# underdoc-wang/STC-GNN

Hardware: AMD Instinct MI355X
Metric: STC-GNN fwd+bwd samples/sec at N=50k,C=32; SpMM HBM GB/s vs peak, 1/8 GPU (higher is better)
Workload: dtype f32; 1 GPU; full STC-GNN train step (fwd + ComboLoss + bwd + grad all-reduce + Adam), csr-fixed, 224x224 queen grid N=50176 nnz=398724, C=32, hidden=16, K=2, layers=2, T=18+6; global_batch=8, batch_per_gpu=8, parallelism=batch-shard x1, operand_format=f16x2, grad_bucket_bytes=88132, grad_large_bytes=0, input_seeds=X, Y: Bernoulli(0.1635), torch seed 1000 + rank

## Files before the change

stc-gnn_amd/csrc/stc_spmm_ring2.hip:

```cpp
#include "stc_spmm_host.h"

namespace {

constexpr int R2_THREADS = 256, R2_WAVES = R2_THREADS / 64;
constexpr int R2_INT = STC_RING2_INTERIOR;
constexpr int R2_L1 = STC_RING2_FIRST;
constexpr int R2_L2 = STC_RING2_SECOND;
constexpr int R2_W = STC_RING2_WIDTH;
constexpr int R2_Q = 32;
constexpr int R2_STAGE = R2_L2 / (2 * R2_WAVES);
constexpr int R2_S1 = R2_L1 / (2 * R2_WAVES);
constexpr int R2_S2 = R2_INT / (2 * R2_WAVES);
constexpr int R2_MAX_ADD = STC_RING2_MAX_ADD;

using v4f = __attribute__((ext_vector_type(4))) float;

struct Ring2Plan {
    const int32_t *l2_rows, *l1_rows, *int_rows;
    const int32_t *t1, *t2;
    int n_patches;
};

struct Ring2Args {
    Ring2Plan pl;
    const v4f *A, *A2;
    const v4f* add[R2_MAX_ADD];
    int n_add;
    const v4f *U, *Cand;
    v4f *Y, *Y2, *Z;
    int n, F4;
    float alpha1, alpha2;
    const v4f* add0[R2_MAX_ADD];
    float scale0[R2_MAX_ADD];
};

enum { R2_SUM = 0, R2_BLEND = 1, R2_CHAIN = 2, R2_BLEND0 = 3 };

__device__ __forceinline__ void lds_only_barrier() { asm volatile("s_waitcnt lgkmcnt(0)\n\ts_barrier" ::: "memory"); }

template <int MODE, bool HAS_A2, int NADD, int N0 = 0>
__global__ __launch_bounds__(R2_THREADS, 2) void ring2_sum_kernel(Ring2Args a) {
    static_assert((MODE != R2_BLEND && MODE != R2_BLEND0) || (NADD == 1 && !HAS_A2), "the blend forms: one addend (A), one gathered operand (Bm)");
    static_assert((MODE == R2_CHAIN) == (N0 > 0), "interior addends: the chain form, at least one");
    extern __shared__ __attribute__((aligned(16))) unsigned char lds[];
    v4f* tile = reinterpret_cast<v4f*>(lds);
    int2* tab1 = reinterpret_cast<int2*>(lds + (size_t)R2_L2 * R2_Q * 16);
    int2* tab2 = tab1 + R2_L1 * R2_W;

    const int p = stc_xcd_tile(blockIdx.x, a.pl.n_patches);
    if (p < 0) return;
    const int b = blockIdx.y;
    const int tid = threadIdx.x, lane = tid & 63, half = lane >> 5, q = lane & 31;
    const int wave = __builtin_amdgcn_readfirstlane(tid >> 6);
    const int hw = wave * 2 + half;
    const int n_chunks = a.F4 / R2_Q;

    for (int e = tid; e < R2_L1 * R2_W; e += R2_THREADS) tab1[e] = reinterpret_cast<const int2*>(a.pl.t1)[(size_t)p * R2_L1 * R2_W + e];
    for (int e = tid; e < R2_INT * R2_W; e += R2_THREADS) tab2[e] = reinterpret_cast<const int2*>(a.pl.t2)[(size_t)p * R2_INT * R2_W + e];

    int stage_row[R2_STAGE], l1_row[R2_S1], in_row[R2_S2];
#pragma unroll
    for (int k = 0; k < R2_STAGE; ++k) stage_row[k] = a.pl.l2_rows[(size_t)p * R2_L2 + k * 8 + hw];
#pragma unroll
    for (int i = 0; i < R2_S1; ++i) l1_row[i] = a.pl.l1_rows[(size_t)p * R2_L1 + i * 8 + hw];
#pragma unroll
    for (int i = 0; i < R2_S2; ++i) in_row[i] = a.pl.int_rows[(size_t)p * R2_INT + i * 8 + hw];

    const unsigned base = (unsigned)b * (unsigned)a.n * (unsigned)a.F4 + (unsigned)q;
    unsigned stage_off[R2_STAGE], l1_off[R2_S1];
#pragma unroll
    for (int k = 0; k < R2_STAGE; ++k) stage_off[k] = base + (unsigned)stage_row[k] * (unsigned)a.F4;
#pragma unroll
    for (int i = 0; i < R2_S1; ++i) l1_off[i] = base + (unsigned)(l1_row[i] >= 0 ? (l1_row[i] & 0x3FFFFFFF) : 0) * (unsigned)a.F4;
    v4f st[R2_STAGE];
    auto request = [&](int chunk) {
#pragma unroll
        for (int k = 0; k < R2_STAGE; ++k) {
            const unsigned at = stage_off[k] + chunk * R2_Q;
            st[k] = a.A[at];
            if (HAS_A2) st[k] += a.A2[at];
        }
    };
    constexpr int NOP = MODE == R2_CHAIN ? NADD : MODE == R2_BLEND0 ? NADD + 1 : NADD + 2, NOPA = NOP > 0 ? NOP : 1;
    auto slot_at = [&](int i, int chunk) { return l1_off[i] + (unsigned)(chunk * R2_Q); };
    auto request_slot = [&](v4f (&o)[NOPA], int i, int chunk) {
        const unsigned at = slot_at(i, chunk);
#pragma unroll
        for (int k = 0; k < NADD; ++k) o[k] = a.add[k][at];
        if constexpr (MODE != R2_CHAIN) {
            o[NADD] = a.U[at];
            if constexpr (MODE != R2_BLEND0) o[NADD + 1] = a.Cand[at];
        }
    };
    v4f opn[NOPA];
    request(0);
    request_slot(opn, 0, 0);
    for (int chunk = 0; chunk < n_chunks; ++chunk) {
        if (chunk) lds_only_barrier();
#pragma unroll
        for (int k = 0; k < R2_STAGE; ++k) tile[(k * 8 + hw) * R2_Q + q] = st[k];
        lds_only_barrier();
        const bool more = chunk + 1 < n_chunks;
        v4f dy[R2_S1];
#pragma unroll
        for (int i = 0; i < R2_S1; ++i) {
            const int slot = i * 8 + hw, row = l1_row[i];
            const bool interior = row >= 0 && (row & (1 << 30));
            v4f cur[NOPA];
#pragma unroll
            for (int k = 0; k < NOP; ++k) cur[k] = opn[k];
            if (i + 1 < R2_S1) {
                request_slot(opn, i + 1, chunk);
            } else if (more) {
                request(chunk + 1);
                request_slot(opn, 0, chunk + 1);
            }
            v4f acc = {0.f, 0.f, 0.f, 0.f};
#pragma unroll
            for (int w = 0; w < R2_W; ++w) {
                const int2 t = tab1[slot * R2_W + w];
                const v4f x = *reinterpret_cast<const v4f*>(lds + t.x + q * 16);
                const float v = __int_as_float(t.y);
#pragma unroll
                for (int c = 0; c < 4; ++c) acc[c] = fmaf(v, x[c], acc[c]);
            }
            v4f dh = MODE == R2_CHAIN ? a.alpha1 * acc : acc;
#pragma unroll
            for (int k = 0; k < NADD; ++k) dh += cur[k];
            if constexpr (MODE == R2_CHAIN) {
                if (a.Y != nullptr && interior) __builtin_nontemporal_store(dh, a.Y + slot_at(i, chunk));
                dy[i] = dh;
            } else if constexpr (MODE == R2_SUM) {
                const v4f u = cur[NOPA - 2], cd = cur[NOPA - 1];
                if (interior) __builtin_nontemporal_store(dh, a.Y + slot_at(i, chunk));
#pragma unroll
                for (int c = 0; c < 4; ++c) dy[i][c] = dh[c] * u[c] * (1.f - cd[c] * cd[c]);
            } else {
                const v4f u = cur[NADD], cd = MODE == R2_BLEND0 ? v4f{0.f, 0.f, 0.f, 0.f} : cur[NOPA - 1];
                v4f cand;
#pragma unroll
                for (int c = 0; c < 4; ++c) {
                    cand[c] = stc_tanh(dh[c]);
                    if constexpr (MODE == R2_BLEND0) dy[i][c] = u[c] * cand[c];
                    else dy[i][c] = (1.f - u[c]) * cd[c] + u[c] * cand[c];
                }
                if (interior) {
                    if (a.Y != nullptr) __builtin_nontemporal_store(cand, a.Y + slot_at(i, chunk));
                    __builtin_nontemporal_store(dy[i], a.Y2 + slot_at(i, chunk));
                }
            }
        }
        lds_only_barrier();
#pragma unroll
        for (int i = 0; i < R2_S1; ++i) tile[(i * 8 + hw) * R2_Q + q] = dy[i];
        v4f own[R2_S2][N0 > 0 ? N0 : 1];
        if constexpr (MODE == R2_CHAIN) {
#pragma unroll
            for (int i = 0; i < R2_S2; ++i)
#pragma unroll
                for (int k = 0; k < N0; ++k)
                    own[i][k] = a.add0[k][base + (unsigned)(in_row[i] >= 0 ? in_row[i] : 0) * (unsigned)a.F4 + (unsigned)(chunk * R2_Q)];
        }
        lds_only_barrier();
#pragma unroll
        for (int i = 0; i < R2_S2; ++i) {
            const int r = i * 8 + hw, row = in_row[i];
            v4f acc = {0.f, 0.f, 0.f, 0.f};
#pragma unroll
            for (int w = 0; w < R2_W; ++w) {
                const int2 t = tab2[r * R2_W + w];
                const v4f x = *reinterpret_cast<const v4f*>(lds + t.x + q * 16);
                const float v = __int_as_float(t.y);
#pragma unroll
                for (int c = 0; c < 4; ++c) acc[c] = fmaf(v, x[c], acc[c]);
            }
            if constexpr (MODE == R2_CHAIN) {
                acc *= a.alpha2;
#pragma unroll
                for (int k = 0; k < N0; ++k) acc += a.scale0[k] * own[i][k];
            }
            if (row >= 0) __builtin_nontemporal_store(acc, a.Z + (base + (unsigned)row * (unsigned)a.F4 + (unsigned)(chunk * R2_Q)));
        }
    }
}

template <int MODE, bool HAS_A2>
int launch_ring2(const Ring2Args& a, int batch, hipStream_t s, int n_add0 = 0) {
    const size_t lds = (size_t)R2_L2 * R2_Q * 16 + (size_t)(R2_L1 + R2_INT) * R2_W * sizeof(int2);
    static_assert((size_t)R2_L2 * R2_Q * 16 + (size_t)(R2_L1 + R2_INT) * R2_W * sizeof(int2) <= 64 * 1024, "within the default dynamic-LDS limit: no attribute to set");
    using Kernel = void (*)(Ring2Args);
    Kernel kern = nullptr;
    if constexpr (MODE == R2_BLEND || MODE == R2_BLEND0) {
        kern = ring2_sum_kernel<MODE, false, 1>;
    } else if constexpr (MODE == R2_CHAIN) {
        static constexpr Kernel table[3][R2_MAX_ADD] = {
#define STC_R2_ROW(NA) {ring2_sum_kernel<R2_CHAIN, HAS_A2, NA, 1>, ring2_sum_kernel<R2_CHAIN, HAS_A2, NA, 2>, ring2_sum_kernel<R2_CHAIN, HAS_A2, NA, 3>, \
                        ring2_sum_kernel<R2_CHAIN, HAS_A2, NA, 4>, ring2_sum_kernel<R2_CHAIN, HAS_A2, NA, 5>}
            STC_R2_ROW(0), STC_R2_ROW(1), STC_R2_ROW(2)};
#undef STC_R2_ROW
        kern = table[a.n_add][n_add0 - 1];
    } else {
        switch (a.n_add) {
            case 0: kern = ring2_sum_kernel<R2_SUM, HAS_A2, 0>; break;
            case 1: kern = ring2_sum_kernel<R2_SUM, HAS_A2, 1>; break;
            case 2: kern = ring2_sum_kernel<R2_SUM, HAS_A2, 2>; break;
            case 3: kern = ring2_sum_kernel<R2_SUM, HAS_A2, 3>; break;
            case 4: kern = ring2_sum_kernel<R2_SUM, HAS_A2, 4>; break;
            default: kern = ring2_sum_kernel<R2_SUM, HAS_A2, 5>; break;
        }
    }
    const int per = (a.pl.n_patches + stc::kNumXcd - 1) / stc::kNumXcd;
    hipLaunchKernelGGL(kern, dim3(per * stc::kNumXcd, batch), dim3(R2_THREADS), lds, s, a);
    return stc::launched("stc_ring2 launch");
}

int check_ring2(const char* who, const void* l2_rows, const void* l1_rows, const void* int_rows, const void* t1, const void* t2, int n_patches, int n_rows,
                int batch, int C, int h) {
    STC_REQUIRE(h == 16 && C >= 1 && (C * h) % (4 * R2_Q) == 0, STC_EUNSUPPORTED, "%s: rows of C * h = %d floats (hidden 16, whole 512-byte chunks)", who, C * h);
    STC_REQUIRE(batch <= 65535 && n_patches >= 0, STC_EINVAL, "%s: bad sizes", who);
    if (int rc = stc::check_state_rows(who, n_rows, batch, C, h, true)) return rc;
    STC_REQUIRE((long long)batch * n_rows * (C * h / 4) < (1ll << 28), STC_ELIMIT, "%s: planes of %lld 16-byte pieces (32-bit offsets: < 2^28)", who,
                (long long)batch * n_rows * (C * h / 4));
    if (batch == 0 || n_rows == 0) return STC_OK;
    STC_REQUIRE(n_patches >= 1 && (long long)n_patches * R2_INT >= n_rows, STC_EINVAL, "%s: %d patches cannot cover %d rows", who, n_patches, n_rows);
    STC_REQUIRE(l2_rows && l1_rows && int_rows && t1 && t2, STC_EINVAL, "%s: null plan array", who);
    STC_REQUIRE(reinterpret_cast<uintptr_t>(t1) % 8 == 0 && reinterpret_cast<uintptr_t>(t2) % 8 == 0, STC_EALIGN, "%s: tables must be 8-byte aligned", who);
    return STC_OK;
}

}

#if !defined(STC_RING2_FIRST_UNIT)

extern "C" int stc_ring2_sum_f32(const int32_t* l2_rows, const int32_t* l1_rows, const int32_t* int_rows, const int32_t* t1, const int32_t* t2,
                                 int32_t n_patches, int32_t n_rows,
                                 const float* A, const float* A2, int32_t n_add, const float* const* add,
                                 const float* U, const float* Cand, float* Y, float* Z,
                                 int32_t batch, int32_t C, int32_t h, void* stream) {
    if (int rc = stc::check_addend_count("stc_ring2_sum_f32", "addend", n_add, 0, R2_MAX_ADD, STC_ELIMIT)) return rc;
    if (int rc = check_ring2("stc_ring2_sum_f32", l2_rows, l1_rows, int_rows, t1, t2, n_patches, n_rows, batch, C, h)) return rc;
    if (batch == 0 || n_rows == 0) return STC_OK;
    STC_REQUIRE(A && U && Cand && Y && Z && (n_add == 0 || add), STC_EINVAL, "stc_ring2_sum_f32: null pointer");
    STC_REQUIRE(stc::aligned16(A) && (!A2 || stc::aligned16(A2)) && stc::aligned16(U) && stc::aligned16(Cand) && stc::aligned16(Y) && stc::aligned16(Z),
                STC_EALIGN, "stc_ring2_sum_f32: planes must be 16-byte aligned");
    STC_REQUIRE(Y != A && Y != A2 && Z != A && Z != A2 && Y != Z && Y != U && Y != Cand && Z != U && Z != Cand, STC_EINVAL,
                "stc_ring2_sum_f32: results must not alias the gathered operands, the first ring's gate planes or each other");
    Ring2Args a{};
    a.pl = Ring2Plan{l2_rows, l1_rows, int_rows, t1, t2, n_patches};
    a.A = reinterpret_cast<const v4f*>(A);
    a.A2 = reinterpret_cast<const v4f*>(A2);
    a.n_add = n_add;
    if (int rc = stc::check_addends("stc_ring2_sum_f32", "addend", add, n_add, Y, Z)) return rc;
    for (int i = 0; i < n_add; ++i) a.add[i] = reinterpret_cast<const v4f*>(add[i]);
    a.U = reinterpret_cast<const v4f*>(U);
    a.Cand = reinterpret_cast<const v4f*>(Cand);
    a.Y = reinterpret_cast<v4f*>(Y);
    a.Z = reinterpret_cast<v4f*>(Z);
    a.n = n_rows;
    a.F4 = C * h / 4;
    hipStream_t s = static_cast<hipStream_t>(stream);
    return A2 ? launch_ring2<R2_SUM, true>(a, batch, s) : launch_ring2<R2_SUM, false>(a, batch, s);
}

extern "C" int stc_ring2_blend_f32(const int32_t* l2_rows, const int32_t* l1_rows, const int32_t* int_rows, const int32_t* t1, const int32_t* t2,
                                   int32_t n_patches, int32_t n_rows,
                                   const float* Bm, const float* A, const float* U, const float* H,
                                   float* Cand, float* Hnew, float* SHnew,
                                   int32_t batch, int32_t C, int32_t h, void* stream) {
    if (int rc = check_ring2("stc_ring2_blend_f32", l2_rows, l1_rows, int_rows, t1, t2, n_patches, n_rows, batch, C, h)) return rc;
    if (batch == 0 || n_rows == 0) return STC_OK;
    STC_REQUIRE(Bm && A && U && H && Hnew && SHnew, STC_EINVAL, "stc_ring2_blend_f32: null pointer");
    for (const void* q : {(const void*)Bm, (const void*)A, (const void*)U, (const void*)H, (const void*)Cand, (const void*)Hnew, (const void*)SHnew})
        STC_REQUIRE(stc::aligned16(q), STC_EALIGN, "stc_ring2_blend_f32: planes must be 16-byte aligned");
    for (const float* out : {Cand, Hnew, SHnew})
        STC_REQUIRE(out != Bm && out != A && out != U && out != H, STC_EINVAL, "stc_ring2_blend_f32: a result aliases an operand (the first ring re-reads them)");
    STC_REQUIRE(Cand != Hnew && Cand != SHnew && Hnew != SHnew, STC_EINVAL, "stc_ring2_blend_f32: results alias each other");
    Ring2Args a{};
    a.pl = Ring2Plan{l2_rows, l1_rows, int_rows, t1, t2, n_patches};
    a.A = reinterpret_cast<const v4f*>(Bm);
    a.n_add = 1;
    a.add[0] = reinterpret_cast<const v4f*>(A);
    a.U = reinterpret_cast<const v4f*>(U);
    a.Cand = reinterpret_cast<const v4f*>(H);
    a.Y = reinterpret_cast<v4f*>(Cand);
    a.Y2 = reinterpret_cast<v4f*>(Hnew);
    a.Z = reinterpret_cast<v4f*>(SHnew);
    a.n = n_rows;
    a.F4 = C * h / 4;
    return launch_ring2<R2_BLEND, false>(a, batch, static_cast<hipStream_t>(stream));
}

extern "C" int stc_ring2_chain_f32(const int32_t* l2_rows, const int32_t* l1_rows, const int32_t* int_rows, const int32_t* t1, const int32_t* t2,
                                   int32_t n_patches, int32_t n_rows,
                                   const float* A, const float* A2, float alpha1, int32_t n_add1, const float* const* add1, float* V,
                                   float alpha2, int32_t n_add0, const float* const* add0, const float* scale0, float* Z,
                                   int32_t batch, int32_t C, int32_t h, void* stream) {
    if (int rc = stc::check_addend_count("stc_ring2_chain_f32", "first-ring addend", n_add1, 0, 2, STC_ELIMIT)) return rc;
    if (int rc = stc::check_addend_count("stc_ring2_chain_f32", "interior addend", n_add0, 1, R2_MAX_ADD, STC_ELIMIT)) return rc;
    if (int rc = check_ring2("stc_ring2_chain_f32", l2_rows, l1_rows, int_rows, t1, t2, n_patches, n_rows, batch, C, h)) return rc;
    if (batch == 0 || n_rows == 0) return STC_OK;
    STC_REQUIRE(A && Z && add0 && (n_add1 == 0 || add1), STC_EINVAL, "stc_ring2_chain_f32: null pointer");
    STC_REQUIRE(stc::aligned16(A) && (!A2 || stc::aligned16(A2)) && (!V || stc::aligned16(V)) && stc::aligned16(Z), STC_EALIGN,
                "stc_ring2_chain_f32: planes must be 16-byte aligned");
    STC_REQUIRE(Z != A && Z != A2 && V != A && (!V || V != A2) && V != Z, STC_EINVAL, "stc_ring2_chain_f32: results must not alias the gathered operands or each other");
    Ring2Args a{};
    a.pl = Ring2Plan{l2_rows, l1_rows, int_rows, t1, t2, n_patches};
    a.A = reinterpret_cast<const v4f*>(A);
    a.A2 = reinterpret_cast<const v4f*>(A2);
    a.n_add = n_add1;
    if (int rc = stc::check_addends("stc_ring2_chain_f32", "first-ring addend", add1, n_add1, Z, V)) return rc;
    if (int rc = stc::check_addends("stc_ring2_chain_f32", "interior addend", add0, n_add0, Z, V)) return rc;
    for (int i = 0; i < n_add1; ++i) a.add[i] = reinterpret_cast<const v4f*>(add1[i]);
    for (int i = 0; i < n_add0; ++i) {
        a.add0[i] = reinterpret_cast<const v4f*>(add0[i]);
        a.scale0[i] = scale0 ? scale0[i] : 1.f;
    }
    a.alpha1 = alpha1;
    a.alpha2 = alpha2;
    a.Y = reinterpret_cast<v4f*>(V);
    a.Z = reinterpret_cast<v4f*>(Z);
    a.n = n_rows;
    a.F4 = C * h / 4;
    hipStream_t s = static_cast<hipStream_t>(stream);
    return A2 ? launch_ring2<R2_CHAIN, true>(a, batch, s, n_add0) : launch_ring2<R2_CHAIN, false>(a, batch, s, n_add0);
}

#else

extern "C" int stc_ring2_blend_first_f32(const int32_t* l2_rows, const int32_t* l1_rows, const int32_t* int_rows, const int32_t* t1, const int32_t* t2,
                                         int32_t n_patches, int32_t n_rows,
                                         const float* Bm, const float* A, const float* U,
                                         float* Cand, float* Hnew, float* SHnew,
                                         int32_t batch, int32_t C, int32_t h, void* stream) {
    if (int rc = check_ring2("stc_ring2_blend_first_f32", l2_rows, l1_rows, int_rows, t1, t2, n_patches, n_rows, batch, C, h)) return rc;
    if (batch == 0 || n_rows == 0) return STC_OK;
    STC_REQUIRE(Bm && A && U && Hnew && SHnew, STC_EINVAL, "stc_ring2_blend_first_f32: null pointer");
    for (const void* q : {(const void*)Bm, (const void*)A, (const void*)U, (const void*)Cand, (const void*)Hnew, (const void*)SHnew})
        STC_REQUIRE(stc::aligned16(q), STC_EALIGN, "stc_ring2_blend_first_f32: planes must be 16-byte aligned");
    for (const float* out : {Cand, Hnew, SHnew})
        STC_REQUIRE(out != Bm && out != A && out != U, STC_EINVAL, "stc_ring2_blend_first_f32: a result aliases an operand (the first ring re-reads them)");
    STC_REQUIRE(Cand != Hnew && Cand != SHnew && Hnew != SHnew, STC_EINVAL, "stc_ring2_blend_first_f32: results alias each other");
    Ring2Args a{};
    a.pl = Ring2Plan{l2_rows, l1_rows, int_rows, t1, t2, n_patches};
    a.A = reinterpret_cast<const v4f*>(Bm);
    a.n_add = 1;
    a.add[0] = reinterpret_cast<const v4f*>(A);
    a.U = reinterpret_cast<const v4f*>(U);
    a.Y = reinterpret_cast<v4f*>(Cand);
    a.Y2 = reinterpret_cast<v4f*>(Hnew);
    a.Z = reinterpret_cast<v4f*>(SHnew);
    a.n = n_rows;
    a.F4 = C * h / 4;
    return launch_ring2<R2_BLEND0, false>(a, batch, static_cast<hipStream_t>(stream));
}

#endif
```

Baseline: 32.97 samples/s.

## Keep ring2 row indices in scalar registers and move next-chunk prefetch after compute

Row indices for the staged, first-ring and interior rows are now loaded with readfirstlane into SGPR pairs and selected per half-wave, so per-row VGPR offsets are no longer precomputed. The per-patch gather tables are held in registers (one or two entries per lane) and written to LDS after the first requests are issued, replacing strided copy loops. The next chunk's prefetch moves from inside the last slot iteration to after a sched_barrier, and the gather loop is factored into a helper. The aim is lower VGPR pressure and better occupancy, at the cost of some scalar address arithmetic and a shorter overlap window for the prefetch.

```diff
diff --git a/stc-gnn_amd/csrc/stc_spmm_ring2.hip b/stc-gnn_amd/csrc/stc_spmm_ring2.hip
--- a/stc-gnn_amd/csrc/stc_spmm_ring2.hip
+++ b/stc-gnn_amd/csrc/stc_spmm_ring2.hip
@@ -38,13 +38,29 @@
 
 __device__ __forceinline__ void lds_only_barrier() { asm volatile("s_waitcnt lgkmcnt(0)\n\ts_barrier" ::: "memory"); }
 
+constexpr int R2_TILE_BYTES = R2_L2 * R2_Q * 16;
+constexpr int R2_LDS_BYTES = R2_TILE_BYTES + (R2_L1 + R2_INT) * R2_W * (int)sizeof(int2);
+
+__device__ __forceinline__ v4f ring2_gather(const unsigned char* lds, const int2* tab, int row, int q) {
+    v4f acc = {0.f, 0.f, 0.f, 0.f};
+#pragma unroll
+    for (int w = 0; w < R2_W; ++w) {
+        const int2 t = tab[row * R2_W + w];
+        const v4f x = *reinterpret_cast<const v4f*>(lds + t.x + q * 16);
+        const float v = __int_as_float(t.y);
+#pragma unroll
+        for (int c = 0; c < 4; ++c) acc[c] = fmaf(v, x[c], acc[c]);
+    }
+    return acc;
+}
+
 template <int MODE, bool HAS_A2, int NADD, int N0 = 0>
 __global__ __launch_bounds__(R2_THREADS, 2) void ring2_sum_kernel(Ring2Args a) {
     static_assert((MODE != R2_BLEND && MODE != R2_BLEND0) || (NADD == 1 && !HAS_A2), "the blend forms: one addend (A), one gathered operand (Bm)");
     static_assert((MODE == R2_CHAIN) == (N0 > 0), "interior addends: the chain form, at least one");
     extern __shared__ __attribute__((aligned(16))) unsigned char lds[];
     v4f* tile = reinterpret_cast<v4f*>(lds);
-    int2* tab1 = reinterpret_cast<int2*>(lds + (size_t)R2_L2 * R2_Q * 16);
+    int2* tab1 = reinterpret_cast<int2*>(lds + R2_TILE_BYTES);
     int2* tab2 = tab1 + R2_L1 * R2_W;
 
     const int p = stc_xcd_tile(blockIdx.x, a.pl.n_patches);
@@ -55,36 +71,39 @@
     const int hw = wave * 2 + half;
     const int n_chunks = a.F4 / R2_Q;
 
-    for (int e = tid; e < R2_L1 * R2_W; e += R2_THREADS) tab1[e] = reinterpret_cast<const int2*>(a.pl.t1)[(size_t)p * R2_L1 * R2_W + e];
-    for (int e = tid; e < R2_INT * R2_W; e += R2_THREADS) tab2[e] = reinterpret_cast<const int2*>(a.pl.t2)[(size_t)p * R2_INT * R2_W + e];
-
-    int stage_row[R2_STAGE], l1_row[R2_S1], in_row[R2_S2];
-#pragma unroll
-    for (int k = 0; k < R2_STAGE; ++k) stage_row[k] = a.pl.l2_rows[(size_t)p * R2_L2 + k * 8 + hw];
-#pragma unroll
-    for (int i = 0; i < R2_S1; ++i) l1_row[i] = a.pl.l1_rows[(size_t)p * R2_L1 + i * 8 + hw];
-#pragma unroll
-    for (int i = 0; i < R2_S2; ++i) in_row[i] = a.pl.int_rows[(size_t)p * R2_INT + i * 8 + hw];
-
+    static_assert(R2_L1 * R2_W == 2 * R2_THREADS && R2_INT * R2_W == R2_THREADS, "table entries per lane: two of the first ring's, one of the interior's");
+    const int2* t1 = reinterpret_cast<const int2*>(a.pl.t1) + (size_t)p * R2_L1 * R2_W;
+    const int2 e1a = t1[tid], e1b = t1[tid + R2_THREADS], e2 = reinterpret_cast<const int2*>(a.pl.t2)[(size_t)p * R2_INT * R2_W + tid];
+
+    int stage_rows[R2_STAGE][2], l1_rows[R2_S1][2], in_rows[R2_S2][2];
+#pragma unroll
+    for (int h2 = 0; h2 < 2; ++h2) {
+#pragma unroll
+        for (int k = 0; k < R2_STAGE; ++k) stage_rows[k][h2] = __builtin_amdgcn_readfirstlane(a.pl.l2_rows[(size_t)p * R2_L2 + k * 8 + wave * 2 + h2]);
+#pragma unroll
+        for (int i = 0; i < R2_S1; ++i) l1_rows[i][h2] = __builtin_amdgcn_readfirstlane(a.pl.l1_rows[(size_t)p * R2_L1 + i * 8 + wave * 2 + h2]);
+#pragma unroll
+        for (int i = 0; i < R2_S2; ++i) in_rows[i][h2] = __builtin_amdgcn_readfirstlane(a.pl.int_rows[(size_t)p * R2_INT + i * 8 + wave * 2 + h2]);
+    }
+    auto pick = [&](const int (&r)[2]) {
+        int r0 = r[0], r1 = r[1];
+        asm volatile("" : "+s"(r0), "+s"(r1));
+        return half ? r1 : r0;
+    };
     const unsigned base = (unsigned)b * (unsigned)a.n * (unsigned)a.F4 + (unsigned)q;
-    unsigned stage_off[R2_STAGE], l1_off[R2_S1];
-#pragma unroll
-    for (int k = 0; k < R2_STAGE; ++k) stage_off[k] = base + (unsigned)stage_row[k] * (unsigned)a.F4;
-#pragma unroll
-    for (int i = 0; i < R2_S1; ++i) l1_off[i] = base + (unsigned)(l1_row[i] >= 0 ? (l1_row[i] & 0x3FFFFFFF) : 0) * (unsigned)a.F4;
     v4f st[R2_STAGE];
     auto request = [&](int chunk) {
 #pragma unroll
         for (int k = 0; k < R2_STAGE; ++k) {
-            const unsigned at = stage_off[k] + chunk * R2_Q;
+            const unsigned at = base + (unsigned)pick(stage_rows[k]) * (unsigned)a.F4 + (unsigned)(chunk * R2_Q);
             st[k] = a.A[at];
             if (HAS_A2) st[k] += a.A2[at];
         }
     };
     constexpr int NOP = MODE == R2_CHAIN ? NADD : MODE == R2_BLEND0 ? NADD + 1 : NADD + 2, NOPA = NOP > 0 ? NOP : 1;
-    auto slot_at = [&](int i, int chunk) { return l1_off[i] + (unsigned)(chunk * R2_Q); };
+    auto slot_at = [&](int row, int chunk) { return base + (unsigned)(row >= 0 ? (row & 0x3FFFFFFF) : 0) * (unsigned)a.F4 + (unsigned)(chunk * R2_Q); };
     auto request_slot = [&](v4f (&o)[NOPA], int i, int chunk) {
-        const unsigned at = slot_at(i, chunk);
+        const unsigned at = slot_at(pick(l1_rows[i]), chunk);
 #pragma unroll
         for (int k = 0; k < NADD; ++k) o[k] = a.add[k][at];
         if constexpr (MODE != R2_CHAIN) {
@@ -95,6 +114,7 @@
     v4f opn[NOPA];
     request(0);
     request_slot(opn, 0, 0);
+    tab1[tid] = e1a, tab1[tid + R2_THREADS] = e1b, tab2[tid] = e2;
     for (int chunk = 0; chunk < n_chunks; ++chunk) {
         if (chunk) lds_only_barrier();
 #pragma unroll
@@ -104,37 +124,24 @@
         v4f dy[R2_S1];
 #pragma unroll
         for (int i = 0; i < R2_S1; ++i) {
-            const int slot = i * 8 + hw, row = l1_row[i];
+            const int slot = i * 8 + hw, row = pick(l1_rows[i]);
             const bool interior = row >= 0 && (row & (1 << 30));
             v4f cur[NOPA];
 #pragma unroll
             for (int k = 0; k < NOP; ++k) cur[k] = opn[k];
-            if (i + 1 < R2_S1) {
-                request_slot(opn, i + 1, chunk);
-            } else if (more) {
-                request(chunk + 1);
-                request_slot(opn, 0, chunk + 1);
-            }
-            v4f acc = {0.f, 0.f, 0.f, 0.f};
-#pragma unroll
-            for (int w = 0; w < R2_W; ++w) {
-                const int2 t = tab1[slot * R2_W + w];
-                const v4f x = *reinterpret_cast<const v4f*>(lds + t.x + q * 16);
-                const float v = __int_as_float(t.y);
-#pragma unroll
-                for (int c = 0; c < 4; ++c) acc[c] = fmaf(v, x[c], acc[c]);
-            }
+            if (i + 1 < R2_S1) request_slot(opn, i + 1, chunk);
+            const v4f acc = ring2_gather(lds, tab1, slot, q);
             v4f dh = MODE == R2_CHAIN ? a.alpha1 * acc : acc;
 #pragma unroll
             for (int k = 0; k < NADD; ++k) dh += cur[k];
             if constexpr (MODE == R2_CHAIN) {
-                if (a.Y != nullptr && interior) __builtin_nontemporal_store(dh, a.Y + slot_at(i, chunk));
+                if (a.Y != nullptr && interior) __builtin_nontemporal_store(dh, a.Y + slot_at(row, chunk));
                 dy[i] = dh;
             } else if constexpr (MODE == R2_SUM) {
                 const v4f u = cur[NOPA - 2], cd = cur[NOPA - 1];
-                if (interior) __builtin_nontemporal_store(dh, a.Y + slot_at(i, chunk));
-#pragma unroll
-                for (int c = 0; c < 4; ++c) dy[i][c] = dh[c] * u[c] * (1.f - cd[c] * cd[c]);
+                if (interior) __builtin_nontemporal_store(dh, a.Y + slot_at(row, chunk));
+#pragma unroll
+                for (int c = 0; c < 4; ++c) dy[i][c] = dh[c] * u[c] * fmaf(-cd[c], cd[c], 1.f);
             } else {
                 const v4f u = cur[NADD], cd = MODE == R2_BLEND0 ? v4f{0.f, 0.f, 0.f, 0.f} : cur[NOPA - 1];
                 v4f cand;
@@ -145,10 +152,16 @@
                     else dy[i][c] = (1.f - u[c]) * cd[c] + u[c] * cand[c];
                 }
                 if (interior) {
-                    if (a.Y != nullptr) __builtin_nontemporal_store(cand, a.Y + slot_at(i, chunk));
-                    __builtin_nontemporal_store(dy[i], a.Y2 + slot_at(i, chunk));
+                    if (a.Y != nullptr) __builtin_nontemporal_store(cand, a.Y + slot_at(row, chunk));
+                    __builtin_nontemporal_store(dy[i], a.Y2 + slot_at(row, chunk));
                 }
             }
+            asm volatile("" : "+v"(dy[i]));
+        }
+        __builtin_amdgcn_sched_barrier(0);
+        if (more) {
+            request(chunk + 1);
+            request_slot(opn, 0, chunk + 1);
         }
         lds_only_barrier();
 #pragma unroll
@@ -159,21 +172,13 @@
             for (int i = 0; i < R2_S2; ++i)
 #pragma unroll
                 for (int k = 0; k < N0; ++k)
-                    own[i][k] = a.add0[k][base + (unsigned)(in_row[i] >= 0 ? in_row[i] : 0) * (unsigned)a.F4 + (unsigned)(chunk * R2_Q)];
+                    own[i][k] = a.add0[k][base + (unsigned)max(pick(in_rows[i]), 0) * (unsigned)a.F4 + (unsigned)(chunk * R2_Q)];
         }
         lds_only_barrier();
 #pragma unroll
         for (int i = 0; i < R2_S2; ++i) {
-            const int r = i * 8 + hw, row = in_row[i];
-            v4f acc = {0.f, 0.f, 0.f, 0.f};
-#pragma unroll
-            for (int w = 0; w < R2_W; ++w) {
-                const int2 t = tab2[r * R2_W + w];
-                const v4f x = *reinterpret_cast<const v4f*>(lds + t.x + q * 16);
-                const float v = __int_as_float(t.y);
-#pragma unroll
-                for (int c = 0; c < 4; ++c) acc[c] = fmaf(v, x[c], acc[c]);
-            }
+            const int r = i * 8 + hw, row = pick(in_rows[i]);
+            v4f acc = ring2_gather(lds, tab2, r, q);
             if constexpr (MODE == R2_CHAIN) {
                 acc *= a.alpha2;
 #pragma unroll
@@ -186,8 +191,8 @@
 
 template <int MODE, bool HAS_A2>
 int launch_ring2(const Ring2Args& a, int batch, hipStream_t s, int n_add0 = 0) {
-    const size_t lds = (size_t)R2_L2 * R2_Q * 16 + (size_t)(R2_L1 + R2_INT) * R2_W * sizeof(int2);
-    static_assert((size_t)R2_L2 * R2_Q * 16 + (size_t)(R2_L1 + R2_INT) * R2_W * sizeof(int2) <= 64 * 1024, "within the default dynamic-LDS limit: no attribute to set");
+    const size_t lds = R2_LDS_BYTES;
+    static_assert(R2_LDS_BYTES <= 64 * 1024, "within the default dynamic-LDS limit: no attribute to set");
     using Kernel = void (*)(Ring2Args);
     Kernel kern = nullptr;
     if constexpr (MODE == R2_BLEND || MODE == R2_BLEND0) {
```

Result: no change. 33.03 samples/s (median of 3 runs) (+0.2%).
